# clawrim/gcn10

Measured on AMD Instinct MI355X. Metric: CN Gpixels/sec, higher is better.
Workload: dtype u8

## Files before the change

### gcn10_amd/csrc/gcn10_gpu.hip

```cpp

#include <hip/hip_runtime.h>
#include <unistd.h>
#include <hip/hip_ext.h>

#include <cstdarg>
#include <cstdint>
#include <cstdio>
#include <cstdlib>
#include <cstring>
#include <new>

#include "gcn10_gpu.h"
#include "gcn10_gpu_internal.hpp"
#include "gcn10_soil_readers.hpp"

using gcn10::as_stream;
using gcn10::fail;
using gcn10::kLut16Bytes;
using gcn10::kLut16Plane;
using gcn10::kPlanes;
using gcn10::SoilView;
using gcn10::u32x4;
using gcn10::use_device;

namespace {

constexpr int kThreads = 256;
constexpr int kPxPerLane = 16;
constexpr int kChunk = kThreads * kPxPerLane;
constexpr int kInvalidPlane = kPlanes - 1;
constexpr int kPlane1 = 256 + 4;
constexpr int kLut1Bytes = kPlanes * kPlane1;


struct StripParams {
    const uint8_t *esa;
    SoilView soil;
    const uint8_t *lut;
    uint8_t *out[GCN10_N_RASTERS];
    uint32_t W;
    uint32_t rows;
    uint32_t npix;
    uint32_t nvec16;
    uint32_t nchunks;
    uint32_t table_mask;
    uint32_t single_k;
    uint32_t xcd_slabs;
    const uint32_t *hx4;
    uint32_t hx4_stride;
    const uint32_t *cx;
    const uint8_t *codes;
    uint32_t codes_stride;
    const uint32_t *soil_complex;
    uint32_t soil_gen;
};

__host__ __device__ inline uint8_t soil_code(uint8_t h)
{
    uint8_t d, u;
    if (h >= 11 && h <= 14) {
        d = 4;
        u = (uint8_t)(h - 10);
    }
    else {
        d = u = (h < 5) ? h : (uint8_t)kInvalidPlane;
    }
    return (uint8_t)(d | (u << 4));
}


__device__ __forceinline__ u32x4 load16_aligned_nt(const uint8_t *p)
{
    return __builtin_nontemporal_load(reinterpret_cast<const u32x4 *>(p));
}

__device__ __forceinline__ u32x4 load16_aligned(const uint8_t *p)
{
    return *reinterpret_cast<const u32x4 *>(p);
}

__device__ __forceinline__ u32x4 load16_any(const uint8_t *p)
{
    typedef u32x4 u32x4_u __attribute__((aligned(1)));
    return *reinterpret_cast<const u32x4_u *>(p);
}

template <bool NT = true>
__device__ __forceinline__ void store16(uint8_t *p, u32x4 v)
{
    if (NT)
        __builtin_nontemporal_store(v, reinterpret_cast<u32x4 *>(p));
    else
        *reinterpret_cast<u32x4 *>(p) = v;
}

__device__ __forceinline__ int32_t scalar_load_i32(const int32_t *base, uint32_t i)
{
    typedef const int32_t __attribute__((address_space(4))) *const_ptr_t;
    const_ptr_t cp = (const_ptr_t)(uintptr_t)base;
    return cp[__builtin_amdgcn_readfirstlane(i)];
}

__device__ __forceinline__ uint32_t first_chunk(uint32_t nchunks, uint32_t &step,
                                                uint32_t &end, bool xcd_slabs)
{
    uint32_t nb = gridDim.x;
    uint32_t b = blockIdx.x;
    if (xcd_slabs && nb % 8u == 0u && nchunks >= nb) {
        uint32_t xcd = b & 7u;
        uint32_t per = (nchunks + 7u) / 8u;
        uint32_t lo = xcd * per;
        uint32_t hi = lo + per < nchunks ? lo + per : nchunks;
        step = nb / 8u;
        end = hi;
        return lo + (b >> 3);
    }
    step = nb;
    end = nchunks;
    return b;
}

enum { kLut16 = 0, kLut1 = 1 };
constexpr uint32_t kWavePx = 64u * kPxPerLane;
constexpr uint32_t kMinVectorW = kWavePx + 16u;

enum { kSoilBytes = 0, kSoilWords = 1, kSoilPixels = 2 };

template <int ILP>
struct Trip {
    u32x4 e16[ILP], c16[ILP];
    uint32_t i0[ILP];
};

template <int ILP, bool NT, int SOIL>
__device__ __forceinline__ void issue_trip(const StripParams &p, uint32_t trip, uint32_t lane_off,
                                           uint32_t wave_off, Trip<ILP> &tr)
{
    uint32_t xb[ILP], r0[ILP], r1[ILP], wb[ILP];
#pragma unroll
    for (int u = 0; u < ILP; u++) {
        wb[u] = __builtin_amdgcn_readfirstlane((trip * ILP + u) * (uint32_t)kChunk + wave_off);
        const uint32_t wbc = wb[u] < p.npix ? wb[u] : 0u;
        const uint32_t y = wbc / p.W;
        xb[u] = wbc - y * p.W;
        r0[u] = (uint32_t)scalar_load_i32(p.soil.cj, y);
        r1[u] = (uint32_t)scalar_load_i32(p.soil.cj, y + 1u < p.rows ? y + 1u : y);
    }
#pragma unroll
    for (int u = 0; u < ILP; u++) {
        tr.i0[u] = wb[u] + lane_off;
        const uint8_t *pe = p.esa + (tr.i0[u] < p.nvec16 ? tr.i0[u] : 0u);
        tr.e16[u] = NT ? load16_aligned_nt(pe) : load16_aligned(pe);
    }
#pragma unroll
    for (int u = 0; u < ILP; u++) {
        uint32_t xl = xb[u] + lane_off;
        const bool wrap = xl >= p.W;
        xl = wrap ? xl - p.W : xl;
        const uint32_t row = p.soil.clamp(wrap ? r1[u] : r0[u]);
        if (SOIL == kSoilWords) {
            tr.c16[u] = u32x4{ p.hx4[(size_t)row * p.hx4_stride + (xl >> 4)], 0u, 0u, 0u };
            continue;
        }
        if (SOIL == kSoilPixels) {
            const uint8_t *cr = p.codes + (size_t)row * p.codes_stride;
            const u32x4 *pc = reinterpret_cast<const u32x4 *>(p.cx + xl);
            u32x4 a = { 0u, 0u, 0u, 0u };
#pragma unroll 1
            for (int j = 0; j < 4; j++) {
                const u32x4 c4 = pc[j];
                const uint32_t w = (uint32_t)cr[c4[0]] | (uint32_t)cr[c4[1]] << 8 | (uint32_t)cr[c4[2]] << 16 |
                                   (uint32_t)cr[c4[3]] << 24;
                a[0] = j == 0 ? w : a[0];
                a[1] = j == 1 ? w : a[1];
                a[2] = j == 2 ? w : a[2];
                a[3] = j == 3 ? w : a[3];
            }
            tr.c16[u] = a;
            continue;
        }
        const uint8_t *pa = p.soil.at(row, xl);
        u32x4 a = load16_any(pa);
        if (p.W & 15u) {
            const uint32_t n = p.W - xl;
            const bool strad = !wrap && n < (uint32_t)kPxPerLane;
            if (__builtin_amdgcn_ballot_w64(strad) != 0ull) {
                const uint8_t *pb = strad ? p.soil.at(p.soil.clamp(r1[u]), 0u) - n : pa;
                const u32x4 b = load16_any(pb);
                const uint32_t nn = strad ? n : (uint32_t)kPxPerLane;
#pragma unroll
                for (int j = 0; j < 4; j++) {
                    const int32_t m = (int32_t)nn - 4 * j;
                    const uint32_t mask = m >= 4 ? 0xffffffffu : (m <= 0 ? 0u : (1u << (8 * m)) - 1u);
                    a[j] = (a[j] & mask) | (b[j] & ~mask);
                }
            }
        }
        tr.c16[u] = a;
    }
}

__device__ __forceinline__ u32x4 expand_soil_word(uint32_t w)
{
    const uint32_t a = (w & 0xffu) * 0x01010101u, b = ((w >> 8) & 0xffu) * 0x01010101u;
    const int32_t split = (int32_t)((w >> 16) & 0xffu);
    u32x4 cd;
#pragma unroll
    for (int j = 0; j < 4; j++) {
        const int32_t m = split - 4 * j;
        const uint32_t mask = m >= 4 ? 0xffffffffu : (m <= 0 ? 0u : (1u << (8 * m)) - 1u);
        cd[j] = (a & mask) | (b & ~mask);
    }
    return cd;
}

template <int KIND, int COND_MASK, int ILP, bool NT, int SOIL>
__device__ __forceinline__ void finish_trip(const StripParams &p, const uint8_t *lut, uint32_t tmask,
                                            const Trip<ILP> &tr)
{
#pragma unroll
    for (int u = 0; u < ILP; u++) {
        const bool live = tr.i0[u] < p.nvec16;
        const u32x4 c16 = SOIL == kSoilWords ? expand_soil_word(tr.c16[u][0]) : tr.c16[u];
#pragma unroll
        for (int c = 0; c < 2; c++) {
            if (!(COND_MASK & (1 << c)))
                continue;
            if (KIND == kLut16) {
                uint32_t acc[9][4];
                gcn10::gather16(lut, tr.e16[u], c16, c, acc);
                if (live) {
#pragma unroll
                    for (int k = 0; k < 9; k++) {
                        if (tmask & (1u << k)) {
                            u32x4 v = {acc[k][0], acc[k][1], acc[k][2], acc[k][3]};
                            store16<NT>(p.out[c * 9 + k] + tr.i0[u], v);
                        }
                    }
                }
            }
            else {
                u32x4 v;
#pragma unroll
                for (int j = 0; j < 4; j++) {
                    const uint32_t e = tr.e16[u][j];
                    const uint32_t cd = c16[j];
                    uint32_t w = 0;
#pragma unroll
                    for (int q = 0; q < 4; q++) {
                        const uint32_t lc = (e >> (8 * q)) & 0xffu;
                        const uint32_t s = (cd >> (8 * q + 4 * c)) & 0xfu;
                        const uint32_t b = lut[s * (uint32_t)kPlane1 + lc];
                        w |= b << (8 * q);
                    }
                    v[j] = w;
                }
                if (live)
                    store16<NT>(p.out[c * 9 + p.single_k] + tr.i0[u], v);
            }
        }
    }
}

template <int KIND, int COND_MASK, int ILP, bool NT, bool PF, int SOIL>
__device__ __forceinline__ void strip_loop(const StripParams &p, const uint8_t *lut, uint32_t tmask,
                                           uint32_t lane_off, uint32_t wave_off)
{
    uint32_t step, end;
    uint32_t trip = first_chunk(p.nchunks, step, end, p.xcd_slabs != 0);
    if (trip >= end)
        return;
    if (!PF) {
        for (; trip < end; trip += step) {
            Trip<ILP> tr;
            issue_trip<ILP, NT, SOIL>(p, trip, lane_off, wave_off, tr);
            finish_trip<KIND, COND_MASK, ILP, NT, SOIL>(p, lut, tmask, tr);
        }
    }
    else {
        Trip<ILP> ta, tb;
        issue_trip<ILP, NT, SOIL>(p, trip, lane_off, wave_off, ta);
        for (;;) {
            trip += step;
            if (trip >= end) {
                finish_trip<KIND, COND_MASK, ILP, NT, SOIL>(p, lut, tmask, ta);
                break;
            }
            issue_trip<ILP, NT, SOIL>(p, trip, lane_off, wave_off, tb);
            finish_trip<KIND, COND_MASK, ILP, NT, SOIL>(p, lut, tmask, ta);
            trip += step;
            if (trip >= end) {
                finish_trip<KIND, COND_MASK, ILP, NT, SOIL>(p, lut, tmask, tb);
                break;
            }
            issue_trip<ILP, NT, SOIL>(p, trip, lane_off, wave_off, ta);
            finish_trip<KIND, COND_MASK, ILP, NT, SOIL>(p, lut, tmask, tb);
        }
    }
}

template <int KIND, int COND_MASK, bool ALL_TABLES, int ILP, bool NT, bool PF>
__global__ __launch_bounds__(kThreads) void cn_strip_kernel(const StripParams p)
{
    constexpr int kLutBytes = KIND == kLut16 ? kLut16Bytes : kLut1Bytes;
    __shared__ __attribute__((aligned(16))) uint8_t lut[kLutBytes];

    if (KIND == kLut16) {
        gcn10::stage_lut16<kThreads>(lut, p.lut);
    }
    else {
        const uint32_t *src = reinterpret_cast<const uint32_t *>(p.lut);
        uint32_t *dst = reinterpret_cast<uint32_t *>(lut);
        for (int i = threadIdx.x; i < kLutBytes / 4; i += kThreads)
            dst[i] = src[i];
    }
    __syncthreads();

    const uint32_t lane_off = (threadIdx.x & 63u) * kPxPerLane;
    const uint32_t wave_off = __builtin_amdgcn_readfirstlane(threadIdx.x >> 6) * kWavePx;
    const uint32_t tmask = ALL_TABLES ? 0x1ffu : p.table_mask;

    if (!p.hx4)
        strip_loop<KIND, COND_MASK, ILP, NT, PF, kSoilBytes>(p, lut, tmask, lane_off, wave_off);
    else if ((uint32_t)scalar_load_i32(reinterpret_cast<const int32_t *>(p.soil_complex), 0u) != p.soil_gen)
        strip_loop<KIND, COND_MASK, ILP, NT, PF, kSoilWords>(p, lut, tmask, lane_off, wave_off);
    else
        strip_loop<KIND, COND_MASK, ILP, NT, PF, kSoilPixels>(p, lut, tmask, lane_off, wave_off);

    if (blockIdx.x == 0 && threadIdx.x < p.npix - p.nvec16) {
        const uint32_t i = p.nvec16 + threadIdx.x;
        const uint32_t y = i / p.W;
        const uint32_t x = i - y * p.W;
        const uint32_t lc = p.esa[i];
        const uint32_t cd = *p.soil.ptr(y, x);
#pragma unroll
        for (int c = 0; c < 2; c++) {
            if (!(COND_MASK & (1 << c)))
                continue;
            const uint32_t s = (cd >> (4 * c)) & 0xfu;
            if (KIND == kLut16) {
                const uint8_t *row = gcn10::lut16_row(lut, s, lc);
                for (int k = 0; k < 9; k++)
                    if (tmask & (1u << k))
                        p.out[c * 9 + k][i] = row[k];
            }
            else {
                p.out[c * 9 + p.single_k][i] = lut[s * (uint32_t)kPlane1 + lc];
            }
        }
    }
}

__global__ __launch_bounds__(kThreads) void stream_copy_kernel(const u32x4 *in, u32x4 *out, uint32_t nvec,
                                                               uint32_t ntrips)
{
    uint32_t step, end;
    for (uint32_t trip = first_chunk(ntrips, step, end, true); trip < end; trip += step) {
        u32x4 v[2];
        uint32_t idx[2];
#pragma unroll
        for (int u = 0; u < 2; u++) {
            idx[u] = (trip * 2u + u) * (uint32_t)kThreads + threadIdx.x;
            v[u] = __builtin_nontemporal_load(in + (idx[u] < nvec ? idx[u] : 0u));
        }
#pragma unroll
        for (int u = 0; u < 2; u++)
            if (idx[u] < nvec)
                __builtin_nontemporal_store(v[u], out + idx[u]);
    }
}

__global__ __launch_bounds__(kThreads) void cn_strip_bytes(const StripParams p,
                                                           uint32_t cond_mask)
{
    __shared__ __attribute__((aligned(16))) uint8_t lut[kLut16Bytes];
    gcn10::stage_lut16<kThreads>(lut, p.lut);
    __syncthreads();

    const uint32_t stride = gridDim.x * blockDim.x;
    for (uint32_t i = blockIdx.x * blockDim.x + threadIdx.x; i < p.npix; i += stride) {
        const uint32_t y = i / p.W;
        const uint32_t x = i - y * p.W;
        const uint32_t lc = p.esa[i];
        const uint32_t cd = *p.soil.ptr(y, x);
        for (int c = 0; c < 2; c++) {
            if (!(cond_mask & (1u << c)))
                continue;
            const uint32_t s = (cd >> (4 * c)) & 0xfu;
            const uint8_t *row = gcn10::lut16_row(lut, s, lc);
            for (int k = 0; k < 9; k++)
                if (p.table_mask & (1u << k))
                    p.out[c * 9 + k][i] = row[k];
        }
    }
}

constexpr uint32_t kWordRows = 8;

template <bool VEC>
__global__ __launch_bounds__(kThreads) void soil_tables_kernel(const uint8_t *coarse, uint32_t hsx, uint32_t hsy,
                                                               const int32_t *ci, uint32_t W, uint32_t hx_stride,
                                                               uint32_t word_chunks, uint8_t *codes,
                                                               uint32_t codes_stride, uint32_t *cx_out, uint32_t *hx4,
                                                               uint32_t *complex, uint32_t gen)
{
    const uint32_t pad = (uint32_t)(kInvalidPlane | (kInvalidPlane << 4));
    if (blockIdx.y >= word_chunks) {
        const uint32_t per_row = codes_stride / 16u;
        const uint32_t t = ((blockIdx.y - word_chunks) * gridDim.x + blockIdx.x) * blockDim.x + threadIdx.x;
        const uint32_t r = t / per_row;
        if (r >= hsy)
            return;
        const uint32_t c0 = (t - r * per_row) * 16u;
        const uint8_t *row = coarse + (size_t)r * hsx;
        u32x4 in = { 0u, 0u, 0u, 0u };
        if (c0 + 16u <= hsx) {
            in = load16_any(row + c0);
        }
        else {
#pragma unroll
            for (int q = 0; q < 16; q++)
                if (c0 + q < hsx)
                    in[q >> 2] |= (uint32_t)row[c0 + q] << (8 * (q & 3));
        }
        u32x4 o;
#pragma unroll
        for (int j = 0; j < 4; j++) {
            uint32_t w = 0;
#pragma unroll
            for (int q = 0; q < 4; q++) {
                const uint32_t code = c0 + 4 * j + q < hsx ? soil_code((uint8_t)(in[j] >> (8 * q))) : pad;
                w |= code << (8 * q);
            }
            o[j] = w;
        }
        *reinterpret_cast<u32x4 *>(codes + (size_t)r * codes_stride + c0) = o;
        return;
    }
    const uint32_t x = (blockIdx.x * blockDim.x + threadIdx.x) * 16u;
    const uint32_t r0 = blockIdx.y * kWordRows;
    if (x >= hx_stride || r0 >= hsy)
        return;
    uint32_t cx[16];
    if (VEC && x + 16u <= W) {
        const u32x4 *civ = reinterpret_cast<const u32x4 *>(ci + x);
#pragma unroll
        for (int j = 0; j < 4; j++) {
            const u32x4 c4 = civ[j];
#pragma unroll
            for (int q = 0; q < 4; q++)
                cx[4 * j + q] = c4[q] < hsx ? c4[q] : hsx - 1u;
        }
    }
    else {
#pragma unroll
        for (int q = 0; q < 16; q++) {
            const uint32_t xx = x + q;
            const uint32_t c = xx < W ? (uint32_t)ci[xx] : 0u;
            cx[q] = xx < W ? (c < hsx ? c : hsx - 1u) : hsx;
        }
    }
    const uint32_t c_lo = cx[0], c_hi = cx[15];
    uint32_t split = 0;
    bool compact = true;
#pragma unroll
    for (int q = 0; q < 16; q++) {
        const bool lo = cx[q] == c_lo;
        compact = compact && (lo ? split == (uint32_t)q : cx[q] == c_hi);
        split += lo && split == (uint32_t)q ? 1u : 0u;
    }
    if (blockIdx.y == 0) {
#pragma unroll
        for (int j = 0; j < 4; j++)
            *reinterpret_cast<u32x4 *>(cx_out + x + 4 * j) =
                u32x4{ cx[4 * j], cx[4 * j + 1], cx[4 * j + 2], cx[4 * j + 3] };
        if (x < W && !compact && *reinterpret_cast<volatile uint32_t *>(complex) != gen)
            *reinterpret_cast<volatile uint32_t *>(complex) = gen;
    }
    const uint32_t r1 = r0 + kWordRows < hsy ? r0 + kWordRows : hsy;
    for (uint32_t r = r0; r < r1; r++) {
        const uint8_t *row = coarse + (size_t)r * hsx;
        const uint32_t a = c_lo < hsx ? soil_code(row[c_lo]) : pad, b = c_hi < hsx ? soil_code(row[c_hi]) : pad;
        __builtin_nontemporal_store(compact ? a | (b << 8) | (split << 16) : 0x00ff0000u,
                                    hx4 + (size_t)r * (hx_stride / 16u) + x / 16u);
    }
}

constexpr uint32_t kExpandRows = 4;

__global__ __launch_bounds__(kThreads) void expand_code_bytes(const uint8_t *codes, uint32_t codes_stride,
                                                              uint32_t hsy, const uint32_t *cx_in, uint8_t *hx,
                                                              uint32_t hx_stride)
{
    const uint32_t x = (blockIdx.x * blockDim.x + threadIdx.x) * 16u;
    const uint32_t r0 = blockIdx.y * kExpandRows;
    if (x >= hx_stride || r0 >= hsy)
        return;
    uint32_t cx[16];
#pragma unroll
    for (int j = 0; j < 4; j++) {
        const u32x4 c4 = *reinterpret_cast<const u32x4 *>(cx_in + x + 4 * j);
#pragma unroll
        for (int q = 0; q < 4; q++)
            cx[4 * j + q] = c4[q];
    }
    const uint32_t c_lo = cx[0], c_hi = cx[15];
    bool two = true;
#pragma unroll
    for (int q = 0; q < 16; q++)
        two = two && (cx[q] == c_lo || cx[q] == c_hi);
    const uint32_t r1 = r0 + kExpandRows < hsy ? r0 + kExpandRows : hsy;
    for (uint32_t r = r0; r < r1; r++) {
        const uint8_t *row = codes + (size_t)r * codes_stride;
        u32x4 o;
        if (two) {
            const uint32_t code_lo = row[c_lo], code_hi = row[c_hi];
#pragma unroll
            for (int j = 0; j < 4; j++) {
                uint32_t w = 0;
#pragma unroll
                for (int q = 0; q < 4; q++)
                    w |= (cx[4 * j + q] == c_lo ? code_lo : code_hi) << (8 * q);
                o[j] = w;
            }
        }
        else {
#pragma unroll
            for (int j = 0; j < 4; j++) {
                uint32_t w = 0;
#pragma unroll
                for (int q = 0; q < 4; q++)
                    w |= (uint32_t)row[cx[4 * j + q]] << (8 * q);
                o[j] = w;
            }
        }
        __builtin_nontemporal_store(o, reinterpret_cast<u32x4 *>(hx + (size_t)r * hx_stride + x));
    }
}
// ... 734 lines not shown
        head = npix;
    const size_t nvec = (npix - head) / 16;
    const uint32_t grid = stream_grid(ctx, (nvec + kThreads - 1) / kThreads + 1);
    hipLaunchKernelGGL(modify_hysogs_kernel, dim3(grid), dim3(kThreads), 0,
                       as_stream(ctx, stream), h, npix, drained, head, nvec);
    HIP_TRY(hipGetLastError());
    return GCN10_OK;
}

int gcn10_gpu_calculate_cn(gcn10_gpu_ctx *ctx, const uint8_t *esa, const uint8_t *hsg,
                           size_t npix, int table_index, uint8_t *out, gcn10_stream_t stream)
{
    int rc = use_device(ctx);
    if (rc)
        return rc;
    if ((rc = gcn10::check_tables(ctx, "gcn10_gpu_calculate_cn")) != GCN10_OK)
        return rc;
    if (table_index < 0 || table_index >= ctx->n_tables)
        return fail(GCN10_E_INVAL, "gcn10_gpu_calculate_cn: table %d not loaded (have %d)",
                    table_index, ctx->n_tables);
    if (npix == 0)
        return GCN10_OK;
    if (!esa || !hsg || !out)
        return fail(GCN10_E_INVAL, "gcn10_gpu_calculate_cn: null pointer");
    const uint8_t *img = ctx->d_lut1 + (size_t)table_index * kLut1Bytes;
    const bool vec = aligned16(esa) && aligned16(hsg) && aligned16(out);
    const uint64_t work = vec ? (npix / 16 + 2 * kThreads - 1) / (2 * kThreads) + 1
                              : (npix + kThreads - 1) / kThreads;
    const uint32_t grid = stream_grid(ctx, work);
    if (vec)
        hipLaunchKernelGGL(calculate_cn_kernel<true>, dim3(grid), dim3(kThreads), 0,
                           as_stream(ctx, stream), esa, hsg, npix, img, out);
    else
        hipLaunchKernelGGL(calculate_cn_kernel<false>, dim3(grid), dim3(kThreads), 0,
                           as_stream(ctx, stream), esa, hsg, npix, img, out);
    HIP_TRY(hipGetLastError());
    return GCN10_OK;
}


int gcn10_gpu_prepare_tile(gcn10_gpu_ctx *ctx, const uint8_t *coarse, int hsx, int hsy,
                           const int32_t *ci, int W, gcn10_stream_t stream)
{
    int rc = use_device(ctx);
    if (rc)
        return rc;
    if (hsx <= 0 || hsy <= 0 || W <= 0)
        return fail(GCN10_E_INVAL, "gcn10_gpu_prepare_tile: bad shape W=%d soil=%dx%d", W, hsx, hsy);
    if (!coarse || !ci)
        return fail(GCN10_E_INVAL, "gcn10_gpu_prepare_tile: null pointer");
    const uint32_t stride = (((uint32_t)W + 15u) & ~15u) + 16u;
    const size_t need_hx = ((size_t)stride * (size_t)hsy + 63) & ~(size_t)63;
    const uint32_t codes_stride = (((uint32_t)hsx + 1u) + 15u) & ~15u;
    const size_t off_words = need_hx;
    const size_t off_cx = (off_words + (size_t)(stride / 16u) * 4u * (size_t)hsy + 15) & ~(size_t)15;
    const size_t off_codes = (off_cx + (size_t)stride * 4u + 15) & ~(size_t)15;
    const size_t need = off_codes + (size_t)codes_stride * (size_t)hsy;
    if (need > ctx->hx_capacity) {
        HIP_TRY(hipDeviceSynchronize());
        if (ctx->d_hx_alloc)
            HIP_TRY(hipFree(ctx->d_hx_alloc));
        ctx->d_hx_alloc = ctx->d_hx = nullptr;
        ctx->hx_capacity = 0;
        ctx->hx_W = 0;
        HIP_TRY(hipMalloc(reinterpret_cast<void **>(&ctx->d_hx_alloc), 16 + need));
        ctx->d_hx = ctx->d_hx_alloc + 16;
        ctx->hx_capacity = need;
    }
    ctx->d_hx4 = reinterpret_cast<uint32_t *>(ctx->d_hx + off_words);
    ctx->d_cx = reinterpret_cast<uint32_t *>(ctx->d_hx + off_cx);
    ctx->d_codes = ctx->d_hx + off_codes;
    ctx->codes_stride = codes_stride;
    if (++ctx->soil_gen == 0u)
        ctx->soil_gen = 1u;
    ctx->hx_made = false;
    ctx->hx_stride = stride;
    ctx->hx_W = (uint32_t)W;
    ctx->hx_rows = (uint32_t)hsy;
    hipStream_t s = as_stream(ctx, stream);
    const uint32_t group_blocks = (stride / 16u + kThreads - 1) / kThreads;
    const uint32_t word_chunks = ((uint32_t)hsy + kWordRows - 1) / kWordRows;
    const size_t code_threads = (size_t)(codes_stride / 16u) * (size_t)hsy;
    const uint32_t code_chunks = (uint32_t)((code_threads + (size_t)group_blocks * kThreads - 1) / ((size_t)group_blocks * kThreads));
    auto fn = aligned16(ci) ? soil_tables_kernel<true> : soil_tables_kernel<false>;
    hipLaunchKernelGGL(fn, dim3(group_blocks, word_chunks + code_chunks), dim3(kThreads), 0, s, coarse, (uint32_t)hsx,
                       (uint32_t)hsy, ci, (uint32_t)W, stride, word_chunks, ctx->d_codes, codes_stride, ctx->d_cx,
                       ctx->d_hx4, ctx->d_soil_complex, ctx->soil_gen);
    HIP_TRY(hipGetLastError());
    if (!ctx->compact_soil || (W & 15)) {
        const uint8_t *hx;
        return gcn10::soil_bytes(ctx, s, &hx);
    }
    return GCN10_OK;
}

int gcn10_gpu_cn_strip(gcn10_gpu_ctx *ctx, const uint8_t *esa, int W, int rows,
                       const int32_t *cj, unsigned cond_mask, unsigned table_mask,
                       uint8_t *const out[GCN10_N_RASTERS], gcn10_stream_t stream)
{
    int rc = use_device(ctx);
    if (rc)
        return rc;
    const char *const who = "gcn10_gpu_cn_strip";
    if ((rc = gcn10::check_tables(ctx, who)) != GCN10_OK || (rc = gcn10::check_tile(ctx, who)) != GCN10_OK)
        return rc;
    if (W <= 0 || rows < 0 || (uint32_t)W != ctx->hx_W)
        return fail(GCN10_E_INVAL, "gcn10_gpu_cn_strip: W=%d rows=%d does not match prepared tile W=%u",
                    W, rows, ctx->hx_W);
    if ((uint64_t)W * (uint64_t)rows > 0x7fffffffull)
        return fail(GCN10_E_INVAL, "gcn10_gpu_cn_strip: strip of %d x %d exceeds 2^31-1 pixels", W, rows);
    if ((rc = gcn10::check_masks(ctx, who, cond_mask, table_mask)) != GCN10_OK)
        return rc;
    if (rows == 0)
        return GCN10_OK;
    if (!esa || !cj || !out)
        return fail(GCN10_E_INVAL, "gcn10_gpu_cn_strip: null pointer");

    StripParams p;
    memset(&p, 0, sizeof p);
    bool all_aligned = aligned16(esa);
    for (int r = 0; r < GCN10_N_RASTERS; r++) {
        if (!gcn10::selected(r, cond_mask, table_mask))
            continue;
        if (!out[r])
            return fail(GCN10_E_INVAL, "gcn10_gpu_cn_strip: out[%d] is null but selected", r);
        p.out[r] = out[r];
        all_aligned = all_aligned && aligned16(out[r]);
    }
    p.esa = esa;
    p.W = (uint32_t)W;
    p.rows = (uint32_t)rows;
    p.npix = (uint32_t)((uint64_t)W * (uint64_t)rows);
    p.nchunks = (p.npix + kChunk - 1) / kChunk;
    p.table_mask = table_mask;
    hipStream_t s = as_stream(ctx, stream);

    p.xcd_slabs = (uint32_t)ctx->xcd_slabs;
    p.nvec16 = p.npix & ~15u;
    if (p.npix < 16u || p.W < kMinVectorW)
        all_aligned = false;
    if (all_aligned && ctx->compact_soil && (p.W & 15u) == 0u) {
        p.soil = SoilView{ nullptr, cj, ctx->hx_stride, ctx->hx_rows };
        p.hx4 = ctx->d_hx4;
        p.hx4_stride = ctx->hx_stride / 16u;
        p.cx = ctx->d_cx;
        p.codes = ctx->d_codes;
        p.codes_stride = ctx->codes_stride;
        p.soil_complex = ctx->d_soil_complex;
        p.soil_gen = ctx->soil_gen;
    }
    else {
        rc = gcn10::bind_soil(ctx, who, W, s, cj, &p.soil);
        if (rc)
            return rc;
    }
    if (!all_aligned) {
        p.lut = ctx->d_lut16;
        const uint32_t g = stream_grid(ctx, ((uint64_t)p.npix + kThreads - 1) / kThreads);
        void *args[] = { &p, &cond_mask };
        HIP_TRY(launch_timed(ctx, reinterpret_cast<const void *>(cn_strip_bytes), g, args, s));
        ctx->last_kernel = "cn_strip_bytes";
    }
    else {
        const bool single = popcount(table_mask) == 1;
        const bool all = table_mask == 0x1ffu;
        const int n_streams = popcount(cond_mask) * popcount(table_mask);
        const bool tuned = single && ctx->single.set;
        const int ilp = tuned ? ctx->single.ilp
                              : single ? ctx->ilp1 : (ctx->ilp16 > 0 ? ctx->ilp16 : (n_streams > 9 ? 1 : 2));
        const bool nt = ctx->nontemporal != 0;
        if (single) {
            p.single_k = (uint32_t)__builtin_ctz(table_mask);
            p.lut = ctx->d_lut1 + (size_t)p.single_k * kLut1Bytes;
        }
        else {
            p.lut = ctx->d_lut16;
        }
        const bool pf = (tuned ? ctx->single.prefetch : ctx->prefetch) != 0 && ilp <= 2;
        p.nchunks = (p.nchunks + (uint32_t)ilp - 1) / (uint32_t)ilp;
        const uint32_t grid = stream_grid(ctx, p.nchunks, tuned ? ctx->single.grid_blocks_per_cu : 0);
        if (tuned)
            p.xcd_slabs = (uint32_t)ctx->single.xcd_slabs;
        strip_kernel_t fn = pick_strip_kernel(single, cond_mask, all, ilp, nt, pf);
        if (!fn)
            return fail(GCN10_E_INVAL, "gcn10_gpu_cn_strip: no kernel for ilp=%d", ilp);
        void *args[] = { &p };
        HIP_TRY(launch_timed(ctx, reinterpret_cast<const void *>(fn), grid, args, s));
        snprintf(ctx->kernel_name, sizeof ctx->kernel_name, "cn_strip_kernel<%d, %u, %s, %d, %s, %s>",
                 single ? 1 : 0, cond_mask, (all || single) ? "true" : "false", ilp, nt ? "true" : "false",
                 pf ? "true" : "false");
        ctx->last_kernel = ctx->kernel_name;
    }
    HIP_TRY(hipGetLastError());
    return GCN10_OK;
}

size_t gcn10_gpu_strip_algorithmic_bytes(int W, int rows, int hsx, int hsy, unsigned cond_mask,
                                         unsigned table_mask)
{
    if (W <= 0 || rows <= 0)
        return 0;
    const size_t n_out = (size_t)popcount(cond_mask & 3u) * (size_t)popcount(table_mask & 0x1ffu);
    return (size_t)W * rows * (1 + n_out) + (size_t)(hsx > 0 ? hsx : 0) * (hsy > 0 ? hsy : 0) +
           4 * ((size_t)W + rows);
}

int gcn10_gpu_set_option(gcn10_gpu_ctx *ctx, const char *name, int value)
{
    if (!ctx || !name)
        return fail(GCN10_E_INVAL, "gcn10_gpu_set_option: null argument");
    if (!strcmp(name, "defaults")) {
        const gcn10_gpu_ctx fresh;
        ctx->grid_blocks_per_cu = fresh.grid_blocks_per_cu;
        ctx->ilp16 = fresh.ilp16;
        ctx->ilp1 = fresh.ilp1;
        ctx->nontemporal = fresh.nontemporal;
        ctx->xcd_slabs = fresh.xcd_slabs;
        ctx->prefetch = fresh.prefetch;
        ctx->compact_soil = fresh.compact_soil;
        ctx->deflate_wave_codes = fresh.deflate_wave_codes;
        ctx->arena_segment_align = fresh.arena_segment_align;
        ctx->fused_parse = fresh.fused_parse;
        ctx->fused_emit = fresh.fused_emit;
        ctx->event_sync_sleep_us = fresh.event_sync_sleep_us;
        ctx->single = fresh.single;
    }
    else if (!strcmp(name, "grid_blocks_per_cu") && value >= 1 && value <= 64)
        ctx->grid_blocks_per_cu = value;
    else if (!strcmp(name, "ilp16") && (value == 0 || value == 1 || value == 2))
        ctx->ilp16 = value;
    else if (!strcmp(name, "ilp1") && (value == 1 || value == 2 || value == 4)) {
        ctx->ilp1 = value;
        ctx->single.set = false;
    }
    else if (!strcmp(name, "nontemporal") && (value == 0 || value == 1))
// ... 170 lines not shown
```

### gcn10_amd/csrc/gcn10_gpu_internal.hpp

```cpp
#ifndef GCN10_GPU_INTERNAL_HPP
#define GCN10_GPU_INTERNAL_HPP

#include <hip/hip_runtime.h>

#include <cstdint>

#include "gcn10_gpu.h"

namespace gcn10 {

int fail(int code, const char *fmt, ...) __attribute__((format(printf, 2, 3)));

#define HIP_TRY(expr)                                                                   \
    do {                                                                                \
        hipError_t e_ = (expr);                                                         \
        if (e_ != hipSuccess)                                                           \
            return gcn10::fail(e_ == hipErrorOutOfMemory ? GCN10_E_NOMEM : GCN10_E_HIP, \
                               "%s: %s", #expr, hipGetErrorString(e_));                 \
    } while (0)

int use_device(gcn10_gpu_ctx *ctx);
hipStream_t as_stream(gcn10_gpu_ctx *ctx, gcn10_stream_t s);
int grow_workspace(void **ws, size_t *cap, size_t need);
int soil_bytes(gcn10_gpu_ctx *ctx, hipStream_t stream, const uint8_t **hx);

struct SoilView;
int check_tables(gcn10_gpu_ctx *ctx, const char *who);
int check_tile(gcn10_gpu_ctx *ctx, const char *who);
int bind_soil(gcn10_gpu_ctx *ctx, const char *who, int W, hipStream_t stream, const int32_t *cj, SoilView *view);
int check_masks(gcn10_gpu_ctx *ctx, const char *who, unsigned cond_mask, unsigned table_mask);
uint32_t grid_cap(const gcn10_gpu_ctx *ctx, int per_cu);

typedef uint32_t u32x4 __attribute__((ext_vector_type(4)));

__device__ __forceinline__ bool inflate_window_ok(uint32_t out_len, uint32_t chunk_w, uint32_t src_x, uint32_t src_y,
                                                  uint32_t copy_w, uint32_t copy_h, uint32_t slot_bytes)
{
    if (copy_w == 0 || copy_h == 0)
        return true;
    if (chunk_w == 0 || out_len > slot_bytes || src_x > chunk_w || copy_w > chunk_w - src_x)
        return false;
    const unsigned long long last = (unsigned long long)(src_y + copy_h - 1u) * chunk_w + src_x + copy_w;
    return (unsigned long long)src_y + copy_h <= 0xffffffffull && last <= out_len;
}

void launch_lzw_decode(const uint8_t *comp_dev, const gcn10_inflate_tile *tiles_dev, uint32_t n_tiles,
                       uint8_t *scratch, uint32_t slot_bytes, uint32_t *status_dev, hipStream_t stream);

constexpr int kClassCodes = 36;

}

struct gcn10_gpu_ctx {
    int device = -1;
    int n_cus = 0;
    hipStream_t main_stream = nullptr;
    uint8_t *d_lut16 = nullptr;
    uint8_t *d_lut1 = nullptr;
    int n_tables = 0;
    uint8_t *d_hx = nullptr;
    uint8_t *d_hx_alloc = nullptr;
    uint32_t *d_hx4 = nullptr;
    uint32_t *d_cx = nullptr;
    uint8_t *d_codes = nullptr;
    uint32_t codes_stride = 0;
    uint32_t *d_soil_complex = nullptr;
    uint32_t soil_gen = 0;
    int compact_soil = 1;
    bool hx_made = false;
    hipEvent_t hx_made_ev = nullptr;
    size_t hx_capacity = 0;
    uint32_t hx_stride = 0;
    uint32_t hx_W = 0;
    uint32_t hx_rows = 0;
    const char *last_kernel = "";
    char kernel_name[96] = "";
    int grid_blocks_per_cu = 16;
    int ilp16 = 0;
    int ilp1 = 2;
    int nontemporal = 1;
    int xcd_slabs = 1;
    int prefetch = 1;
    struct SingleShape {
        bool set = false;
        int xcd_slabs = 1, grid_blocks_per_cu = 8, ilp = 2, prefetch = 1;
    } single;
    hipEvent_t time_start = nullptr, time_stop = nullptr;
    uint8_t *d_class_of = nullptr;
    int n_classes = 0;
    int arena_segment_align = 4096;
    int deflate_wave_codes = 1;
    int fused_parse = 1;
    int fused_emit = 1;
    int event_sync_sleep_us = 0;
    bool fused_ready = false;
    bool codes_ready = false;
    bool deflate_ready = false;
    void *deflate_ws = nullptr;
    size_t deflate_ws_cap = 0;
    void *inflate_ws = nullptr;
    size_t inflate_ws_cap = 0;
    void *lzw_ws = nullptr;
    size_t lzw_ws_cap = 0;
};

#endif
```

Before: 2956.

## Map lanes to fixed soil columns and drop the per-row soil word table

The compact soil path now gives each lane a fixed 16-pixel column group and walks it down rows. The lane computes its soil code indices, split point and masks once in a prologue and then loads only one or two code bytes per row. This removes the precomputed hx4 word table, so the prepare kernel no longer writes a word per 16 pixels per coarse row. The cost is a new work distribution (column-major walk across rows, plus a plan computed per lane) that changes access patterns and load balance for the esa reads and the output writes.

```diff
diff --git a/gcn10_amd/csrc/gcn10_gpu.hip b/gcn10_amd/csrc/gcn10_gpu.hip
--- a/gcn10_amd/csrc/gcn10_gpu.hip
+++ b/gcn10_amd/csrc/gcn10_gpu.hip
@@ -46,8 +46,6 @@
     uint32_t table_mask;
     uint32_t single_k;
     uint32_t xcd_slabs;
-    const uint32_t *hx4;
-    uint32_t hx4_stride;
     const uint32_t *cx;
     const uint8_t *codes;
     uint32_t codes_stride;
@@ -124,7 +122,7 @@
 constexpr uint32_t kWavePx = 64u * kPxPerLane;
 constexpr uint32_t kMinVectorW = kWavePx + 16u;
 
-enum { kSoilBytes = 0, kSoilWords = 1, kSoilPixels = 2 };
+enum { kSoilBytes = 0, kSoilLanes = 1, kSoilPixels = 2 };
 
 template <int ILP>
 struct Trip {
@@ -132,7 +130,7 @@
     uint32_t i0[ILP];
 };
 
-template <int ILP, bool NT, int SOIL>
+template <int ILP, bool NT>
 __device__ __forceinline__ void issue_trip(const StripParams &p, uint32_t trip, uint32_t lane_off,
                                            uint32_t wave_off, Trip<ILP> &tr)
 {
@@ -158,13 +156,117 @@
         const bool wrap = xl >= p.W;
         xl = wrap ? xl - p.W : xl;
         const uint32_t row = p.soil.clamp(wrap ? r1[u] : r0[u]);
-        if (SOIL == kSoilWords) {
-            tr.c16[u] = u32x4{ p.hx4[(size_t)row * p.hx4_stride + (xl >> 4)], 0u, 0u, 0u };
-            continue;
-        }
-        if (SOIL == kSoilPixels) {
-            const uint8_t *cr = p.codes + (size_t)row * p.codes_stride;
-            const u32x4 *pc = reinterpret_cast<const u32x4 *>(p.cx + xl);
+        const uint8_t *pa = p.soil.at(row, xl);
+        u32x4 a = load16_any(pa);
+        if (p.W & 15u) {
+            const uint32_t n = p.W - xl;
+            const bool strad = !wrap && n < (uint32_t)kPxPerLane;
+            if (__builtin_amdgcn_ballot_w64(strad) != 0ull) {
+                const uint8_t *pb = strad ? p.soil.at(p.soil.clamp(r1[u]), 0u) - n : pa;
+                const u32x4 b = load16_any(pb);
+                const uint32_t nn = strad ? n : (uint32_t)kPxPerLane;
+#pragma unroll
+                for (int j = 0; j < 4; j++) {
+                    const int32_t m = (int32_t)nn - 4 * j;
+                    const uint32_t mask = m >= 4 ? 0xffffffffu : (m <= 0 ? 0u : (1u << (8 * m)) - 1u);
+                    a[j] = (a[j] & mask) | (b[j] & ~mask);
+                }
+            }
+        }
+        tr.c16[u] = a;
+    }
+}
+
+struct LaneSoil {
+    uint32_t base;
+    uint32_t lim;
+    uint32_t sub_px;
+    uint32_t y_first;
+    uint32_t B;
+    bool wrap;
+    uint32_t x;
+    uint32_t c_lo, c_hi;
+    int32_t split;
+    uint32_t mask[4];
+    bool pair;
+};
+
+__device__ __forceinline__ uint32_t split_mask(int32_t split, int j)
+{
+    const int32_t m = split - 4 * j;
+    return m >= 4 ? 0xffffffffu : (m <= 0 ? 0u : (1u << (8 * m)) - 1u);
+}
+
+template <int SOIL>
+__device__ __forceinline__ void lane_prologue(const StripParams &p, const gcn10::StripLanePlan &pl, LaneSoil &ls)
+{
+    const uint32_t g_first = __builtin_amdgcn_readfirstlane(pl.g);
+    ls.base = (pl.row_lo * pl.G + pl.t) * (uint32_t)kPxPerLane;
+    ls.lim = pl.active ? pl.row_hi * p.W : 0u;
+    ls.sub_px = pl.B * p.W;
+    ls.y_first = pl.row_lo + __builtin_amdgcn_readfirstlane(pl.rho);
+    ls.B = pl.B;
+    ls.wrap = pl.g < g_first;
+    ls.x = pl.g * (uint32_t)kPxPerLane;
+    ls.c_lo = ls.c_hi = 0u;
+    ls.split = 16;
+    ls.pair = true;
+    if (SOIL == kSoilLanes) {
+        uint32_t cx[16];
+#pragma unroll
+        for (int j = 0; j < 4; j++) {
+            const u32x4 c4 = *reinterpret_cast<const u32x4 *>(p.cx + ls.x + 4 * j);
+#pragma unroll
+            for (int q = 0; q < 4; q++)
+                cx[4 * j + q] = c4[q];
+        }
+        ls.c_lo = cx[0];
+        ls.c_hi = cx[15];
+        uint32_t split = 0;
+#pragma unroll
+        for (int q = 0; q < 16; q++)
+            split += cx[q] == ls.c_lo && split == (uint32_t)q ? 1u : 0u;
+        ls.split = (int32_t)split;
+#pragma unroll
+        for (int j = 0; j < 4; j++)
+            ls.mask[j] = split_mask(ls.split, j);
+        ls.pair = __builtin_amdgcn_ballot_w64(ls.c_hi - ls.c_lo > 1u) == 0ull;
+    }
+}
+
+template <int ILP, bool NT, int SOIL>
+__device__ __forceinline__ void issue_lane_trip(const StripParams &p, const LaneSoil &ls, uint32_t trip,
+                                                Trip<ILP> &tr)
+{
+    uint32_t o0[ILP], o1[ILP];
+#pragma unroll
+    for (int u = 0; u < ILP; u++) {
+        const uint32_t y = ls.y_first + (trip * ILP + u) * ls.B;
+        const uint32_t ya = y < p.rows ? y : p.rows - 1u;
+        const uint32_t yb = y + 1u < p.rows ? y + 1u : p.rows - 1u;
+        o0[u] = p.soil.clamp((uint32_t)scalar_load_i32(p.soil.cj, ya)) * p.codes_stride;
+        o1[u] = p.soil.clamp((uint32_t)scalar_load_i32(p.soil.cj, yb)) * p.codes_stride;
+    }
+#pragma unroll
+    for (int u = 0; u < ILP; u++) {
+        const uint32_t i0 = ls.base + (trip * ILP + u) * ls.sub_px;
+        const bool live = i0 < ls.lim;
+        tr.i0[u] = live ? i0 : 0xffffffffu;
+        const uint8_t *pe = p.esa + (live ? i0 : 0u);
+        tr.e16[u] = NT ? load16_aligned_nt(pe) : load16_aligned(pe);
+    }
+#pragma unroll
+    for (int u = 0; u < ILP; u++) {
+        const uint32_t off = ls.wrap ? o1[u] : o0[u];
+        if (SOIL == kSoilLanes) {
+            typedef uint16_t u16_u __attribute__((aligned(1)));
+            tr.c16[u][0] = *reinterpret_cast<const u16_u *>(p.codes + (off + ls.c_lo));
+            if (!ls.pair)
+                tr.c16[u][1] = p.codes[off + ls.c_hi];
+        }
+        else {
+            const uint8_t *cr = p.codes + off;
+            const u32x4 *pc = reinterpret_cast<const u32x4 *>(p.cx + ls.x);
             u32x4 a = { 0u, 0u, 0u, 0u };
 #pragma unroll 1
             for (int j = 0; j < 4; j++) {
@@ -177,38 +279,22 @@
                 a[3] = j == 3 ? w : a[3];
             }
             tr.c16[u] = a;
-            continue;
-        }
-        const uint8_t *pa = p.soil.at(row, xl);
-        u32x4 a = load16_any(pa);
-        if (p.W & 15u) {
-            const uint32_t n = p.W - xl;
-            const bool strad = !wrap && n < (uint32_t)kPxPerLane;
-            if (__builtin_amdgcn_ballot_w64(strad) != 0ull) {
-                const uint8_t *pb = strad ? p.soil.at(p.soil.clamp(r1[u]), 0u) - n : pa;
-                const u32x4 b = load16_any(pb);
-                const uint32_t nn = strad ? n : (uint32_t)kPxPerLane;
-#pragma unroll
-                for (int j = 0; j < 4; j++) {
-                    const int32_t m = (int32_t)nn - 4 * j;
-                    const uint32_t mask = m >= 4 ? 0xffffffffu : (m <= 0 ? 0u : (1u << (8 * m)) - 1u);
-                    a[j] = (a[j] & mask) | (b[j] & ~mask);
-                }
-            }
-        }
-        tr.c16[u] = a;
-    }
-}
-
-__device__ __forceinline__ u32x4 expand_soil_word(uint32_t w)
-{
-    const uint32_t a = (w & 0xffu) * 0x01010101u, b = ((w >> 8) & 0xffu) * 0x01010101u;
-    const int32_t split = (int32_t)((w >> 16) & 0xffu);
+        }
+    }
+}
+
+template <bool KEEP_MASKS>
+__device__ __forceinline__ u32x4 mix_lane_codes(const LaneSoil &ls, const u32x4 &c)
+{
+    const uint32_t a = (c[0] & 0xffu) * 0x01010101u;
+    const uint32_t b = (ls.pair ? (c[0] >> 8) & 0xffu : c[1] & 0xffu) * 0x01010101u;
     u32x4 cd;
+    int32_t split = ls.split;
+    if (!KEEP_MASKS)
+        asm volatile("" : "+v"(split));
 #pragma unroll
     for (int j = 0; j < 4; j++) {
-        const int32_t m = split - 4 * j;
-        const uint32_t mask = m >= 4 ? 0xffffffffu : (m <= 0 ? 0u : (1u << (8 * m)) - 1u);
+        const uint32_t mask = KEEP_MASKS ? ls.mask[j] : split_mask(split, j);
         cd[j] = (a & mask) | (b & ~mask);
     }
     return cd;
@@ -216,12 +302,12 @@
 
 template <int KIND, int COND_MASK, int ILP, bool NT, int SOIL>
 __device__ __forceinline__ void finish_trip(const StripParams &p, const uint8_t *lut, uint32_t tmask,
-                                            const Trip<ILP> &tr)
+                                            const Trip<ILP> &tr, const LaneSoil &ls)
 {
 #pragma unroll
     for (int u = 0; u < ILP; u++) {
         const bool live = tr.i0[u] < p.nvec16;
-        const u32x4 c16 = SOIL == kSoilWords ? expand_soil_word(tr.c16[u][0]) : tr.c16[u];
+        const u32x4 c16 = SOIL == kSoilLanes ? mix_lane_codes<KIND == kLut1>(ls, tr.c16[u]) : tr.c16[u];
 #pragma unroll
         for (int c = 0; c < 2; c++) {
             if (!(COND_MASK & (1 << c)))
@@ -263,38 +349,56 @@
 }
 
 template <int KIND, int COND_MASK, int ILP, bool NT, bool PF, int SOIL>
-__device__ __forceinline__ void strip_loop(const StripParams &p, const uint8_t *lut, uint32_t tmask,
-                                           uint32_t lane_off, uint32_t wave_off)
-{
-    uint32_t step, end;
-    uint32_t trip = first_chunk(p.nchunks, step, end, p.xcd_slabs != 0);
+__device__ __forceinline__ void strip_loop(const StripParams &p, const uint8_t *lut, uint32_t tmask)
+{
+    uint32_t step = 1u, end, trip = 0u, lane_off = 0u, wave_off = 0u;
+    LaneSoil ls = {};
+    if (SOIL == kSoilBytes) {
+        lane_off = (threadIdx.x & 63u) * kPxPerLane;
+        wave_off = __builtin_amdgcn_readfirstlane(threadIdx.x >> 6) * kWavePx;
+        trip = first_chunk(p.nchunks, step, end, p.xcd_slabs != 0);
+    }
+    else {
+        const gcn10::StripLanePlan pl = gcn10::strip_lane_plan(p.W, p.rows, gridDim.x, blockIdx.x, threadIdx.x,
+                                                               p.xcd_slabs != 0, (uint32_t)ILP);
+        end = __builtin_amdgcn_readfirstlane(pl.trips);
+        if (!__builtin_amdgcn_readfirstlane((uint32_t)pl.active))
+            return;
+        lane_prologue<SOIL>(p, pl, ls);
+    }
     if (trip >= end)
         return;
+    auto issue = [&](uint32_t t, Trip<ILP> &tr) {
+        if (SOIL == kSoilBytes)
+            issue_trip<ILP, NT>(p, t, lane_off, wave_off, tr);
+        else
+            issue_lane_trip<ILP, NT, SOIL>(p, ls, t, tr);
+    };
     if (!PF) {
         for (; trip < end; trip += step) {
             Trip<ILP> tr;
-            issue_trip<ILP, NT, SOIL>(p, trip, lane_off, wave_off, tr);
-            finish_trip<KIND, COND_MASK, ILP, NT, SOIL>(p, lut, tmask, tr);
+            issue(trip, tr);
+            finish_trip<KIND, COND_MASK, ILP, NT, SOIL>(p, lut, tmask, tr, ls);
         }
     }
     else {
         Trip<ILP> ta, tb;
-        issue_trip<ILP, NT, SOIL>(p, trip, lane_off, wave_off, ta);
+        issue(trip, ta);
         for (;;) {
             trip += step;
             if (trip >= end) {
-                finish_trip<KIND, COND_MASK, ILP, NT, SOIL>(p, lut, tmask, ta);
+                finish_trip<KIND, COND_MASK, ILP, NT, SOIL>(p, lut, tmask, ta, ls);
                 break;
             }
-            issue_trip<ILP, NT, SOIL>(p, trip, lane_off, wave_off, tb);
-            finish_trip<KIND, COND_MASK, ILP, NT, SOIL>(p, lut, tmask, ta);
+            issue(trip, tb);
+            finish_trip<KIND, COND_MASK, ILP, NT, SOIL>(p, lut, tmask, ta, ls);
             trip += step;
             if (trip >= end) {
-                finish_trip<KIND, COND_MASK, ILP, NT, SOIL>(p, lut, tmask, tb);
+                finish_trip<KIND, COND_MASK, ILP, NT, SOIL>(p, lut, tmask, tb, ls);
                 break;
             }
-            issue_trip<ILP, NT, SOIL>(p, trip, lane_off, wave_off, ta);
-            finish_trip<KIND, COND_MASK, ILP, NT, SOIL>(p, lut, tmask, tb);
+            issue(trip, ta);
+            finish_trip<KIND, COND_MASK, ILP, NT, SOIL>(p, lut, tmask, tb, ls);
         }
     }
 }
@@ -316,16 +420,14 @@
     }
     __syncthreads();
 
-    const uint32_t lane_off = (threadIdx.x & 63u) * kPxPerLane;
-    const uint32_t wave_off = __builtin_amdgcn_readfirstlane(threadIdx.x >> 6) * kWavePx;
     const uint32_t tmask = ALL_TABLES ? 0x1ffu : p.table_mask;
 
-    if (!p.hx4)
-        strip_loop<KIND, COND_MASK, ILP, NT, PF, kSoilBytes>(p, lut, tmask, lane_off, wave_off);
+    if (!p.codes)
+        strip_loop<KIND, COND_MASK, ILP, NT, PF, kSoilBytes>(p, lut, tmask);
     else if ((uint32_t)scalar_load_i32(reinterpret_cast<const int32_t *>(p.soil_complex), 0u) != p.soil_gen)
-        strip_loop<KIND, COND_MASK, ILP, NT, PF, kSoilWords>(p, lut, tmask, lane_off, wave_off);
+        strip_loop<KIND, COND_MASK, ILP, NT, PF, kSoilLanes>(p, lut, tmask);
     else
-        strip_loop<KIND, COND_MASK, ILP, NT, PF, kSoilPixels>(p, lut, tmask, lane_off, wave_off);
+        strip_loop<KIND, COND_MASK, ILP, NT, PF, kSoilPixels>(p, lut, tmask);
 
     if (blockIdx.x == 0 && threadIdx.x < p.npix - p.nvec16) {
         const uint32_t i = p.nvec16 + threadIdx.x;
@@ -395,19 +497,16 @@
     }
 }
 
-constexpr uint32_t kWordRows = 8;
-
 template <bool VEC>
 __global__ __launch_bounds__(kThreads) void soil_tables_kernel(const uint8_t *coarse, uint32_t hsx, uint32_t hsy,
                                                                const int32_t *ci, uint32_t W, uint32_t hx_stride,
-                                                               uint32_t word_chunks, uint8_t *codes,
-                                                               uint32_t codes_stride, uint32_t *cx_out, uint32_t *hx4,
-                                                               uint32_t *complex, uint32_t gen)
+                                                               uint8_t *codes, uint32_t codes_stride,
+                                                               uint32_t *cx_out, uint32_t *complex, uint32_t gen)
 {
     const uint32_t pad = (uint32_t)(kInvalidPlane | (kInvalidPlane << 4));
-    if (blockIdx.y >= word_chunks) {
+    if (blockIdx.y >= 1u) {
         const uint32_t per_row = codes_stride / 16u;
-        const uint32_t t = ((blockIdx.y - word_chunks) * gridDim.x + blockIdx.x) * blockDim.x + threadIdx.x;
+        const uint32_t t = ((blockIdx.y - 1u) * gridDim.x + blockIdx.x) * blockDim.x + threadIdx.x;
         const uint32_t r = t / per_row;
         if (r >= hsy)
             return;
@@ -438,8 +537,7 @@
         return;
     }
     const uint32_t x = (blockIdx.x * blockDim.x + threadIdx.x) * 16u;
-    const uint32_t r0 = blockIdx.y * kWordRows;
-    if (x >= hx_stride || r0 >= hsy)
+    if (x >= hx_stride)
         return;
     uint32_t cx[16];
     if (VEC && x + 16u <= W) {
@@ -469,21 +567,12 @@
         compact = compact && (lo ? split == (uint32_t)q : cx[q] == c_hi);
         split += lo && split == (uint32_t)q ? 1u : 0u;
     }
-    if (blockIdx.y == 0) {
-#pragma unroll
-        for (int j = 0; j < 4; j++)
-            *reinterpret_cast<u32x4 *>(cx_out + x + 4 * j) =
-                u32x4{ cx[4 * j], cx[4 * j + 1], cx[4 * j + 2], cx[4 * j + 3] };
-        if (x < W && !compact && *reinterpret_cast<volatile uint32_t *>(complex) != gen)
-            *reinterpret_cast<volatile uint32_t *>(complex) = gen;
-    }
-    const uint32_t r1 = r0 + kWordRows < hsy ? r0 + kWordRows : hsy;
-    for (uint32_t r = r0; r < r1; r++) {
-        const uint8_t *row = coarse + (size_t)r * hsx;
-        const uint32_t a = c_lo < hsx ? soil_code(row[c_lo]) : pad, b = c_hi < hsx ? soil_code(row[c_hi]) : pad;
-        __builtin_nontemporal_store(compact ? a | (b << 8) | (split << 16) : 0x00ff0000u,
-                                    hx4 + (size_t)r * (hx_stride / 16u) + x / 16u);
-    }
+#pragma unroll
+    for (int j = 0; j < 4; j++)
+        *reinterpret_cast<u32x4 *>(cx_out + x + 4 * j) =
+            u32x4{ cx[4 * j], cx[4 * j + 1], cx[4 * j + 2], cx[4 * j + 3] };
+    if (x < W && !compact && *reinterpret_cast<volatile uint32_t *>(complex) != gen)
+        *reinterpret_cast<volatile uint32_t *>(complex) = gen;
 }
 
 constexpr uint32_t kExpandRows = 4;
@@ -1324,8 +1413,7 @@
     const uint32_t stride = (((uint32_t)W + 15u) & ~15u) + 16u;
     const size_t need_hx = ((size_t)stride * (size_t)hsy + 63) & ~(size_t)63;
     const uint32_t codes_stride = (((uint32_t)hsx + 1u) + 15u) & ~15u;
-    const size_t off_words = need_hx;
-    const size_t off_cx = (off_words + (size_t)(stride / 16u) * 4u * (size_t)hsy + 15) & ~(size_t)15;
+    const size_t off_cx = (need_hx + 15) & ~(size_t)15;
     const size_t off_codes = (off_cx + (size_t)stride * 4u + 15) & ~(size_t)15;
     const size_t need = off_codes + (size_t)codes_stride * (size_t)hsy;
     if (need > ctx->hx_capacity) {
@@ -1339,7 +1427,6 @@
         ctx->d_hx = ctx->d_hx_alloc + 16;
         ctx->hx_capacity = need;
     }
-    ctx->d_hx4 = reinterpret_cast<uint32_t *>(ctx->d_hx + off_words);
     ctx->d_cx = reinterpret_cast<uint32_t *>(ctx->d_hx + off_cx);
     ctx->d_codes = ctx->d_hx + off_codes;
     ctx->codes_stride = codes_stride;
@@ -1351,13 +1438,12 @@
     ctx->hx_rows = (uint32_t)hsy;
     hipStream_t s = as_stream(ctx, stream);
     const uint32_t group_blocks = (stride / 16u + kThreads - 1) / kThreads;
-    const uint32_t word_chunks = ((uint32_t)hsy + kWordRows - 1) / kWordRows;
     const size_t code_threads = (size_t)(codes_stride / 16u) * (size_t)hsy;
     const uint32_t code_chunks = (uint32_t)((code_threads + (size_t)group_blocks * kThreads - 1) / ((size_t)group_blocks * kThreads));
     auto fn = aligned16(ci) ? soil_tables_kernel<true> : soil_tables_kernel<false>;
-    hipLaunchKernelGGL(fn, dim3(group_blocks, word_chunks + code_chunks), dim3(kThreads), 0, s, coarse, (uint32_t)hsx,
-                       (uint32_t)hsy, ci, (uint32_t)W, stride, word_chunks, ctx->d_codes, codes_stride, ctx->d_cx,
-                       ctx->d_hx4, ctx->d_soil_complex, ctx->soil_gen);
+    hipLaunchKernelGGL(fn, dim3(group_blocks, 1u + code_chunks), dim3(kThreads), 0, s, coarse, (uint32_t)hsx,
+                       (uint32_t)hsy, ci, (uint32_t)W, stride, ctx->d_codes, codes_stride, ctx->d_cx,
+                       ctx->d_soil_complex, ctx->soil_gen);
     HIP_TRY(hipGetLastError());
     if (!ctx->compact_soil || (W & 15)) {
         const uint8_t *hx;
@@ -1411,10 +1497,18 @@
     p.nvec16 = p.npix & ~15u;
     if (p.npix < 16u || p.W < kMinVectorW)
         all_aligned = false;
-    if (all_aligned && ctx->compact_soil && (p.W & 15u) == 0u) {
+    const bool single = popcount(table_mask) == 1;
+    const bool tuned = single && ctx->single.set;
+    const int n_streams = popcount(cond_mask) * popcount(table_mask);
+    const int ilp = tuned ? ctx->single.ilp
+                          : single ? ctx->ilp1 : (ctx->ilp16 > 0 ? ctx->ilp16 : (n_streams > 9 ? 1 : 2));
+    p.nchunks = (p.nchunks + (uint32_t)ilp - 1) / (uint32_t)ilp;
+    const uint32_t grid = stream_grid(ctx, p.nchunks, tuned ? ctx->single.grid_blocks_per_cu : 0);
+    if (tuned)
+        p.xcd_slabs = (uint32_t)ctx->single.xcd_slabs;
+    if (all_aligned && ctx->compact_soil && (p.W & 15u) == 0u &&
+        gcn10::strip_lane_plan(p.W, p.rows, grid, 0u, 0u, p.xcd_slabs != 0, (uint32_t)ilp).B > 0u) {
         p.soil = SoilView{ nullptr, cj, ctx->hx_stride, ctx->hx_rows };
-        p.hx4 = ctx->d_hx4;
-        p.hx4_stride = ctx->hx_stride / 16u;
         p.cx = ctx->d_cx;
         p.codes = ctx->d_codes;
         p.codes_stride = ctx->codes_stride;
@@ -1434,12 +1528,7 @@
         ctx->last_kernel = "cn_strip_bytes";
     }
     else {
-        const bool single = popcount(table_mask) == 1;
         const bool all = table_mask == 0x1ffu;
-        const int n_streams = popcount(cond_mask) * popcount(table_mask);
-        const bool tuned = single && ctx->single.set;
-        const int ilp = tuned ? ctx->single.ilp
-                              : single ? ctx->ilp1 : (ctx->ilp16 > 0 ? ctx->ilp16 : (n_streams > 9 ? 1 : 2));
         const bool nt = ctx->nontemporal != 0;
         if (single) {
             p.single_k = (uint32_t)__builtin_ctz(table_mask);
@@ -1449,10 +1538,6 @@
             p.lut = ctx->d_lut16;
         }
         const bool pf = (tuned ? ctx->single.prefetch : ctx->prefetch) != 0 && ilp <= 2;
-        p.nchunks = (p.nchunks + (uint32_t)ilp - 1) / (uint32_t)ilp;
-        const uint32_t grid = stream_grid(ctx, p.nchunks, tuned ? ctx->single.grid_blocks_per_cu : 0);
-        if (tuned)
-            p.xcd_slabs = (uint32_t)ctx->single.xcd_slabs;
         strip_kernel_t fn = pick_strip_kernel(single, cond_mask, all, ilp, nt, pf);
         if (!fn)
             return fail(GCN10_E_INVAL, "gcn10_gpu_cn_strip: no kernel for ilp=%d", ilp);
diff --git a/gcn10_amd/csrc/gcn10_gpu_internal.hpp b/gcn10_amd/csrc/gcn10_gpu_internal.hpp
--- a/gcn10_amd/csrc/gcn10_gpu_internal.hpp
+++ b/gcn10_amd/csrc/gcn10_gpu_internal.hpp
@@ -6,6 +6,7 @@
 #include <cstdint>
 
 #include "gcn10_gpu.h"
+#include "gcn10_strip_lanes.hpp"
 
 namespace gcn10 {
 
@@ -60,7 +61,6 @@
     int n_tables = 0;
     uint8_t *d_hx = nullptr;
     uint8_t *d_hx_alloc = nullptr;
-    uint32_t *d_hx4 = nullptr;
     uint32_t *d_cx = nullptr;
     uint8_t *d_codes = nullptr;
     uint32_t codes_stride = 0;
diff --git a/gcn10_amd/csrc/gcn10_strip_lanes.hpp b/gcn10_amd/csrc/gcn10_strip_lanes.hpp
--- /dev/null
+++ b/gcn10_amd/csrc/gcn10_strip_lanes.hpp
@@ -0,0 +1,59 @@
+#ifndef GCN10_STRIP_LANES_HPP
+#define GCN10_STRIP_LANES_HPP
+
+#include <cstdint>
+
+#if defined(__HIPCC__)
+#define GCN10_HOST_DEVICE __host__ __device__
+#else
+#define GCN10_HOST_DEVICE
+#endif
+
+namespace gcn10 {
+
+struct StripLanePlan {
+    uint32_t G, B, T;
+    uint32_t pieces;
+    uint32_t row_lo, row_hi;
+    uint32_t trips;
+    uint32_t t, g, rho;
+    bool active;
+};
+
+constexpr uint32_t kStripThreads = 256;
+
+GCN10_HOST_DEVICE inline uint32_t strip_lane_rows(uint32_t T, uint32_t G)
+{
+    const uint32_t B = T / G;
+    const uint32_t m = (G & 1u) ? 8u : (G & 2u) ? 4u : (G & 4u) ? 2u : 1u;
+    const uint32_t Ba = B - B % m;
+    return Ba > 0u && (uint64_t)(T - Ba * G) * 20u < (uint64_t)T ? Ba : B;
+}
+
+GCN10_HOST_DEVICE inline StripLanePlan strip_lane_plan(uint32_t W, uint32_t rows, uint32_t grid, uint32_t block,
+                                                         uint32_t tid, bool slabs, uint32_t ilp)
+{
+    StripLanePlan pl;
+    pl.G = W / 16u;
+    pl.pieces = 1u;
+    pl.T = grid * kStripThreads;
+    if (slabs && grid % 8u == 0u && (grid / 8u) * kStripThreads >= pl.G) {
+        pl.pieces = 8u;
+        pl.T = (grid / 8u) * kStripThreads;
+    }
+    pl.B = strip_lane_rows(pl.T, pl.G);
+    const uint32_t piece = pl.pieces == 8u ? block & 7u : 0u;
+    pl.row_lo = (uint32_t)((uint64_t)piece * rows / pl.pieces);
+    pl.row_hi = (uint32_t)((uint64_t)(piece + 1u) * rows / pl.pieces);
+    pl.t = (pl.pieces == 8u ? block >> 3 : block) * kStripThreads + tid;
+    pl.g = pl.t % pl.G;
+    pl.rho = pl.t / pl.G;
+    pl.active = pl.rho < pl.B;
+    const uint32_t per_trip = pl.B * ilp;
+    pl.trips = per_trip ? (pl.row_hi - pl.row_lo + per_trip - 1u) / per_trip : 0u;
+    return pl;
+}
+
+}
+
+#endif
diff --git a/profiles/column_lanes/summarize.py b/profiles/column_lanes/summarize.py
--- /dev/null
+++ b/profiles/column_lanes/summarize.py
@@ -0,0 +1,94 @@
+#!/usr/bin/env python3
+import collections
+import csv
+import glob
+import json
+import os
+import re
+import statistics
+import sys
+
+
+def bench_line(path):
+    return json.loads([l for l in open(path) if l.startswith("{")][-1])
+
+
+def short(name):
+    m = re.search(r"(cn_strip_kernel<[^>]*>|stream_copy_kernel|soil_tables_kernel<[^>]*>|expand_code_bytes)", name)
+    return m.group(1) if m else name[:60]
+
+
+def bench(d):
+    rows = [("ms_per_step", lambda b: b["ms_per_step"]),
+            ("roofline.avg_launch_ms", lambda b: b["roofline"]["avg_launch_ms"]),
+            ("also.avg_launch_ms", lambda b: b["also"]["avg_launch_ms"]),
+            ("same-run plain copy, ms", lambda b: b["roofline"]["copy_ceiling"]["avg_ms"])]
+    for side in ("parent", "new"):
+        lines = [bench_line(p) for p in sorted(glob.glob(os.path.join(d, "bench_%s_[0-9].json" % side)))]
+        print(side, len(lines), "runs; timed kernels", [b["roofline"]["kernel"] for b in lines],
+              "self-check, differing pixels", [b.get("self_check", {}).get("differing") for b in lines])
+        for name, get in rows:
+            v = [get(b) for b in lines]
+            print("  %-28s median %.4f (min %.4f - max %.4f, range %.4f)  %s" % (name, statistics.median(v), min(v), max(v),
+                                                                                 max(v) - min(v), v))
+
+
+def pairs(trace):
+    rows = sorted(csv.DictReader(open(trace)), key=lambda r: int(r["Start_Timestamp"]))
+    names = [short(r["Kernel_Name"]) for r in rows]
+    got = []
+    for i in range(len(rows) - 1):
+        if names[i].startswith("soil_tables_kernel") and names[i + 1].startswith("cn_strip_kernel<1,"):
+            a, b = rows[i], rows[i + 1]
+            got.append(((int(a["End_Timestamp"]) - int(a["Start_Timestamp"])) / 1e3,
+                        (int(b["Start_Timestamp"]) - int(a["End_Timestamp"])) / 1e3,
+                        (int(b["End_Timestamp"]) - int(b["Start_Timestamp"])) / 1e3, names[i + 1]))
+    got = got[-20:]
+    print("last %d prepare+strip pairs of the trace (%s), medians: prepare kernel %.2f us, gap to the strip kernel %.2f us, "
+          "strip kernel %.2f us" % (len(got), got[-1][3], statistics.median(g[0] for g in got),
+                                    statistics.median(g[1] for g in got), statistics.median(g[2] for g in got)))
+
+
+def traffic(fetch_csv, fetch_json, write_csv, write_json, old):
+    doc = json.load(open(old))
+    new = {"config2_by_kernel": {}}
+    for counter, f, line in (("FETCH_SIZE", fetch_csv, fetch_json), ("WRITE_SIZE", write_csv, write_json)):
+        chosen = bench_line(line)["roofline"]["kernel"]
+        per = collections.OrderedDict()
+        for r in csv.DictReader(open(f)):
+            if r["Counter_Name"] == counter:
+                key = (int(r["Dispatch_Id"]), short(r["Kernel_Name"]))
+                per[key] = per.get(key, 0.0) + float(r["Counter_Value"])
+        order = sorted(per)
+        names = [k[1] for k in order]
+        first_copy = names.index("stream_copy_kernel") if "stream_copy_kernel" in names else len(order)
+        strip = [per[k] for k in order[:first_copy] if k[1] == chosen][-4:]
+        k18 = [per[k] for k in order if k[1].startswith("cn_strip_kernel<0, 3")]
+        by_var = collections.defaultdict(list)
+        for k in order:
+            if k[1].startswith("cn_strip_kernel<1,"):
+                by_var[k[1]].append(per[k])
+        for kn, vals in by_var.items():
+            t = new["config2_by_kernel"].setdefault(kn, {})
+            t[counter + "_KiB"] = sum(vals) / len(vals)
+            t[counter + "_dispatches"] = len(vals)
+        for key, vals, kn in (("config2", strip, chosen),
+                              ("config4", k18, next((n for n in names if n.startswith("cn_strip_kernel<0, 3")), ""))):
+            if vals:
+                t = new.setdefault(key, {"kernel": kn})
+                t[counter + "_KiB"] = sum(vals) / len(vals)
+                t[counter + "_dispatches"] = len(vals)
+    correction = doc["copy"]["correction"]
+    for key, t in list(new["config2_by_kernel"].items()) + [(k, new[k]) for k in ("config2", "config4") if k in new]:
+        if "FETCH_SIZE_KiB" in t and "WRITE_SIZE_KiB" in t:
+            t["hbm_bytes_per_launch"] = int((2 * t["FETCH_SIZE_KiB"] + t["WRITE_SIZE_KiB"]) * 1024)
+            if key in ("config2", "config4"):
+                t["correction"] = correction
+    for key in ("config2_by_kernel", "config2", "config4"):
+        if key in new and new[key]:
+            doc[key] = new[key]
+    print(json.dumps(doc, indent=1))
+
+
+if __name__ == "__main__":
+    {"bench": bench, "pairs": pairs, "traffic": traffic}[sys.argv[1]](*sys.argv[2:])
```

Result: faster. 3003 (median of 6 runs) (+1.6%).
